# 3dlg-hcvc/tricolo

Measured on AMD Instinct MI355X. Metric: trimodal training samples/sec (32^3 voxel + 6-view), higher is better.
Workload: dtype f16 (f16 activation storage + f16 MFMA operands, fp32 accumulate; bf16x3 heads/GRU; within 1e-3 of the fp32 reference)

## Files before the change

### tricolo_amd/csrc/conv_igemm.hip

```cpp
#include "common.h"
#include <stdio.h>
#include <stdlib.h>
#include <map>
#include <mutex>
#include "../../include/tricolo_hip.h"
#include "conv_vox.h"
#include "conv_frag.h"

struct ConvArgs {
    const void* in;
    const void* w_hi;
    const void* w_lo;
    void* out;
    const uint8_t* row_mask;
    const int* row_pos;
    const int* row_count;
    const float* bias;
    float* stats;
    float* slab;
    int B, ID, IH, IW, Cin;
    int OD, OH, OW, Cout;
    int KD, KH, KW, stride, pd, ph, pw;
    int transposed, act, accumulate;
    int Kpad, M, ntaps, cin_shift, ksplit, steps_per_split;
// ... 1248 lines not shown
    HR_FIRST_READS(0u)
    HSTAMP(3);

#pragma unroll 1
    for (;;) {
        const int ng = grp_n(c_g);
        const bool last_chunk = c_chunk == nchunks - 1;
        HR_ELEM(0)
        HR_ELEM(1)
        HR_ELEM(2)
        HR_ELEM(3)
        int n_g = c_g, n_chunk = c_chunk + 1;
        if (n_chunk == nchunks) { n_chunk = 0; n_g += NTLE; }
        if (n_g >= n_my) break;
        if (!STREAM && !w_once) {
            asm volatile("s_waitcnt lgkmcnt(0)" ::: "memory");
            __builtin_amdgcn_s_barrier();
            asm volatile("" ::: "memory");
            w_row_pieces(n_chunk, 0, 0, 6);
            w_row_pieces(n_chunk, 1, 0, 6);
            w_row_pieces(n_chunk, 2, 0, 6);
            asm volatile("s_waitcnt vmcnt(0)" ::: "memory");
            __builtin_amdgcn_s_barrier();
            asm volatile("" ::: "memory");
            const unsigned sb0 = c_sbuf * slab_bytes;
            HR_FIRST_READS(sb0)
        }
        c_g = n_g; c_chunk = n_chunk;
    }
    asm volatile("s_waitcnt lgkmcnt(0)" ::: "memory");
    if (DRIP && d_on) {
#pragma unroll
        for (int d = 0; d < 4; ++d) {
            const v4i q = *(const v4i*)((const char*)red + wave * 4096 + (d >> 1) * 2048 + ((d & 1) * 8 + (lane >> 3)) * 128 +
                                        (((lane & 7) ^ ((((d & 1) * 8 + (lane >> 3)) >> 1) & 7)) << 4));
            if (d_m0 + d * 8 < d_npos) *(v4i*)(d_ptr + d * d_step) = q;
        }
    }
    __syncthreads();
    if (p.stats) halo_store_stats<TN, BN>(cs, cq, red, p.stats, p.Cout, bid / NT, bid % NT, wave, fr, fq, t, false);
    HSTAMP(11);
#ifdef HALO_STAMPS
    if (wave == 0) {
        asm volatile("s_waitcnt lgkmcnt(0)" ::: "memory");
        for (int i = lane; i < 255; i += 64) p.h_dbg[(size_t)blockIdx.x * 256 + i] = i < n_stamp ? stl[i] : 0;
        if (lane == 0) p.h_dbg[(size_t)blockIdx.x * 256 + 255] = n_stamp;
    }
#endif
#undef HR_ELEM
#undef HR_FIRST_READS
#undef HR_ROW
#undef HR_DRIP_READ
#undef HR_DRIP_STORE
#undef HR_KSTEP
#undef HR_MMA
}


#define STEM_MAX_KH 8
struct StemGeom { int TH, slab_rows, row_bytes, ptiles, tiles_per_img, ntiles, grid, npt; };
template <int KH, int NPT, typename AT>
__global__ __launch_bounds__(256, NPT == 2 ? 2 : 1) void conv_stem_kernel(const ConvArgs p, const StemGeom sg) {
    typedef Mma<typename OpOf<AT>::E> MM;
    typedef typename MM::v8 v8;
    extern __shared__ __attribute__((aligned(16))) char smem[];
    const int t = threadIdx.x, lane = t & 63, wave = __builtin_amdgcn_readfirstlane(t >> 6), fr = lane & 15, fq = lane >> 4;
    const int slab_bytes = sg.slab_rows * sg.row_bytes;
    float* const red = (float*)(smem + 2 * slab_bytes);
    const int OW = p.OW, IW = p.IW, IH = p.IH, OH = p.OH;
    const int pt_per_row = OW >> 4;

    v8 wf[KH][4];
    {
        const uint16_t* w = (const uint16_t*)p.w_hi;
#pragma unroll
        for (int kh = 0; kh < KH; ++kh)
#pragma unroll
            for (int ct = 0; ct < 4; ++ct) {
                const uint16_t* src = w + (size_t)(ct * 16 + fr) * p.Kpad + (kh * p.KW + 2 * fq) * 4;
                uint2 lo = make_uint2(0u, 0u), hi = make_uint2(0u, 0u);
                if (2 * fq < p.KW) lo = *(const uint2*)src;
                if (2 * fq + 1 < p.KW) hi = *(const uint2*)(src + 4);
                const uint4 raw = make_uint4(lo.x, lo.y, hi.x, hi.y);
                wf[kh][ct] = __builtin_bit_cast(v8, raw);
            }
        asm volatile("s_waitcnt vmcnt(0)" ::: "memory");
#pragma unroll
        for (int kh = 0; kh < KH; ++kh)
#pragma unroll
            for (int ct = 0; ct < 4; ++ct) asm volatile("" : "+v"(wf[kh][ct]));
    }
    for (int i = t * 16; i < 2 * slab_bytes; i += 256 * 16) *(uint4*)(smem + i) = make_uint4(0u, 0u, 0u, 0u);
    __syncthreads();

    constexpr int MAXLD = 4;
    const int ld_per_row = IW >> 1, nld = sg.slab_rows * ld_per_row;
    int ld_row[MAXLD], ld_goff[MAXLD], ld_loff[MAXLD];
#pragma unroll
    for (int u = 0; u < MAXLD; ++u) {
        const int e = t + u * 256;
        const int srow = e / ld_per_row, xp = e - srow * ld_per_row;
        ld_row[u] = e < nld ? srow : -(1 << 20);
        ld_goff[u] = (srow * IW + 2 * xp) * 8;
        ld_loff[u] = srow * sg.row_bytes + (2 * xp + p.pw) * 8;
    }
    uint4 pre[MAXLD];
    auto fetch = [&](int tile) {
        const int img = tile / sg.tiles_per_img, oh0 = (tile - img * sg.tiles_per_img) * sg.TH;
        const int iy0 = oh0 * 2 - p.ph;
        const char* base = (const char*)p.in + ((size_t)img * IH + iy0) * IW * 8;
#pragma unroll
        for (int u = 0; u < MAXLD; ++u) {
            pre[u] = make_uint4(0u, 0u, 0u, 0u);
            if ((unsigned)(iy0 + ld_row[u]) < (unsigned)IH) pre[u] = *(const uint4*)(base + ld_goff[u]);
        }
    };
    auto stash = [&](int buf) {
        char* sb = smem + buf * slab_bytes;
#pragma unroll
        for (int u = 0; u < MAXLD; ++u)
            if (ld_row[u] >= 0) {
                char* d = sb + ld_loff[u];
                *(uint2*)d = make_uint2(pre[u].x, pre[u].y);
                *(uint2*)(d + 8) = make_uint2(pre[u].z, pre[u].w);
            }
    };

    f32x4 cs[4], cq[4];
#pragma unroll
    for (int ct = 0; ct < 4; ++ct) { cs[ct] = (f32x4){0.f, 0.f, 0.f, 0.f}; cq[ct] = cs[ct]; }
    int boff[NPT], ooff[NPT], orow[NPT];
    bool inside[NPT];
#pragma unroll
    for (int j = 0; j < NPT; ++j) {
        const int q = wave + 4 * j;
        const int qc = q < sg.ptiles ? q : 0;
        const int r = qc / pt_per_row, c0 = (qc - r * pt_per_row) * 16;
        inside[j] = q < sg.ptiles;
        orow[j] = r;
        boff[j] = (2 * r) * sg.row_bytes + (c0 + fr + fq) * 16;
        ooff[j] = ((r * OW) + c0 + fr) * p.Cout + fq * 4;
    }

    int tile = blockIdx.x, buf = 0;
    if (tile < sg.ntiles) { fetch(tile); stash(0); }
    __syncthreads();
    for (; tile < sg.ntiles; tile += gridDim.x) {
        const int nxt = tile + gridDim.x;
        if (nxt < sg.ntiles && !(p.h_abl & 8)) fetch(nxt);
        const char* sb = smem + buf * slab_bytes;
        const int img = tile / sg.tiles_per_img, oh0 = (tile - img * sg.tiles_per_img) * sg.TH;
        f32x4 acc[NPT][4];
#pragma unroll
        for (int j = 0; j < NPT; ++j)
#pragma unroll
            for (int ct = 0; ct < 4; ++ct) acc[j][ct] = (f32x4){0.f, 0.f, 0.f, 0.f};
        if (!(p.h_abl & 1))
#pragma unroll
        for (int kh = 0; kh < KH; ++kh) {
            v8 b[NPT];
#pragma unroll
            for (int j = 0; j < NPT; ++j) b[j] = *(const v8*)(sb + boff[j] + kh * sg.row_bytes);
#pragma unroll
            for (int j = 0; j < NPT; ++j)
#pragma unroll
                for (int ct = 0; ct < 4; ++ct) acc[j][ct] = MM::mma(wf[kh][ct], b[j], acc[j][ct]);
        }
        AT* const obase = (AT*)p.out + ((size_t)img * OH + oh0) * OW * p.Cout;
#pragma unroll
        for (int j = 0; j < NPT; ++j) {
            if (inside[j] && oh0 + orow[j] < OH) {
                AT* o = obase + ooff[j];
#pragma unroll
                for (int ct = 0; ct < 4; ++ct) {
                    f32x4 v = acc[j][ct];
                    if (!(p.h_abl & 4)) Act<AT>::st4(o + ct * 16, make_float4(v[0], v[1], v[2], v[3]));
                    if (p.stats) {
                        v[0] = Act<AT>::rnd(v[0]); v[1] = Act<AT>::rnd(v[1]); v[2] = Act<AT>::rnd(v[2]); v[3] = Act<AT>::rnd(v[3]);
                        cs[ct] += v;
                        cq[ct] += v * v;
                    }
                }
            }
        }
        if (nxt < sg.ntiles) stash(buf ^ 1);
        __syncthreads();
        buf ^= 1;
    }
    if (p.stats) {
#pragma unroll
        for (int ct = 0; ct < 4; ++ct)
#pragma unroll
            for (int r = 0; r < 4; ++r) {
                float s_ = cs[ct][r], q_ = cq[ct][r];
                stat_row_sum(s_, q_);
                stat_stage(red, wave, 64, ct * 16 + fq * 4 + r, fr, s_, q_);
            }
        __syncthreads();
        if (t < 64) {
            float s_, q_;
            stat_wave_sum<4>(red, 0, 64, t, s_, q_);
            stat_store(p.stats, blockIdx.x, p.Cout, 0, t, s_, q_);
        }
    }
}

template <typename AT>
__global__ __launch_bounds__(256) void conv_splitk_finish_kernel(const ConvArgs p) {
    __shared__ float red[16][64][2];
    const int t = threadIdx.x, tc = t & 15, rl = t >> 4;
    const int chunk = blockIdx.x, m0 = chunk * 32, n = blockIdx.y * 64 + tc * 4;
    float4 s4 = make_float4(0.f, 0.f, 0.f, 0.f), q4 = s4;
    const float4 bv = p.bias ? *(const float4*)(p.bias + n) : make_float4(0.f, 0.f, 0.f, 0.f);
    const int Meff = p.row_count ? min(*p.row_count, p.M) : p.M;
#pragma unroll
    for (int rr = 0; rr < 2; ++rr) {
        int m = m0 + rl * 2 + rr;
        if (m >= Meff) continue;
        const size_t pos = p.row_pos ? (size_t)p.row_pos[m] : (size_t)m;
        bool live = p.row_mask ? (p.row_mask[pos] != 0) : true;
        float4 v = make_float4(0.f, 0.f, 0.f, 0.f);
        if (live) {
            const float* sp = p.slab + (size_t)m * p.Cout + n;
            const size_t zs = (size_t)p.M * p.Cout;
            int z = 0;
            for (; z + 4 <= p.ksplit; z += 4) {
                const float4 x0 = *(const float4*)(sp + (size_t)z * zs), x1 = *(const float4*)(sp + (size_t)(z + 1) * zs);
                const float4 x2 = *(const float4*)(sp + (size_t)(z + 2) * zs), x3 = *(const float4*)(sp + (size_t)(z + 3) * zs);
                v.x += x0.x; v.y += x0.y; v.z += x0.z; v.w += x0.w;
                v.x += x1.x; v.y += x1.y; v.z += x1.z; v.w += x1.w;
                v.x += x2.x; v.y += x2.y; v.z += x2.z; v.w += x2.w;
                v.x += x3.x; v.y += x3.y; v.z += x3.z; v.w += x3.w;
            }
            for (; z < p.ksplit; ++z) {
                const float4 x = *(const float4*)(sp + (size_t)z * zs);
                v.x += x.x; v.y += x.y; v.z += x.z; v.w += x.w;
            }
            v.x += bv.x; v.y += bv.y; v.z += bv.z; v.w += bv.w;
            if (p.act == 1) { v.x = fmaxf(v.x, 0.f); v.y = fmaxf(v.y, 0.f); v.z = fmaxf(v.z, 0.f); v.w = fmaxf(v.w, 0.f); }
            else if (p.act == 2) { v.x = tanhf(v.x); v.y = tanhf(v.y); v.z = tanhf(v.z); v.w = tanhf(v.w); }
        }
        AT* o = (AT*)p.out + pos * p.Cout + n;
        if (p.accumulate) { float4 e = Act<AT>::ld4(o); v.x += e.x; v.y += e.y; v.z += e.z; v.w += e.w; }
        Act<AT>::st4(o, v);
        if (sizeof(AT) == 2) v = make_float4(Act<AT>::rnd(v.x), Act<AT>::rnd(v.y), Act<AT>::rnd(v.z), Act<AT>::rnd(v.w));
        s4.x += v.x; s4.y += v.y; s4.z += v.z; s4.w += v.w;
        q4.x += v.x * v.x; q4.y += v.y * v.y; q4.z += v.z * v.z; q4.w += v.w * v.w;
    }
    if (p.stats) {
        float* d = &red[rl][tc * 4][0];
        d[0] = s4.x; d[1] = q4.x; d[2] = s4.y; d[3] = q4.y; d[4] = s4.z; d[5] = q4.z; d[6] = s4.w; d[7] = q4.w;
        __syncthreads();
        if (t < 64) {
            float s = 0.f, q = 0.f;
#pragma unroll
            for (int w = 0; w < 16; ++w) { s += red[w][t][0]; q += red[w][t][1]; }
            p.stats[((size_t)chunk * 2 + 0) * p.Cout + blockIdx.y * 64 + t] = s;
            p.stats[((size_t)chunk * 2 + 1) * p.Cout + blockIdx.y * 64 + t] = q;
        }
    }
}

__device__ __forceinline__ void prep_store(bool f16, uint16_t* hi, bf16_t* lo, size_t idx, float v) {
    if (f16) { hi[idx] = __builtin_bit_cast(uint16_t, (f16_t)v); return; }
    const bf16_t h = (bf16_t)v;
    hi[idx] = __builtin_bit_cast(uint16_t, h);
    if (lo) lo[idx] = (bf16_t)(v - (float)h);
}

__device__ __forceinline__ size_t prep_index(bool frag, int row, int k, int kpad) {
    if (!frag) return (size_t)row * kpad + k;
    return ((size_t)(row >> 4) * (kpad >> 5) + (k >> 5)) * 512 + ((((k & 31) >> 3) * 16 + (row & 15)) << 3) + (k & 7);
}

__device__ __forceinline__ void prep_store4(bool f16, uint16_t* hi, bf16_t* lo, size_t idx, float4 v) {
    if (f16) {
        f16x4 h;
        h[0] = (f16_t)v.x; h[1] = (f16_t)v.y; h[2] = (f16_t)v.z; h[3] = (f16_t)v.w;
        *(f16x4*)(hi + idx) = h;
        return;
    }
    bf16x4 h;
    h[0] = (bf16_t)v.x; h[1] = (bf16_t)v.y; h[2] = (bf16_t)v.z; h[3] = (bf16_t)v.w;
    *(bf16x4*)(hi + idx) = h;
    if (lo) {
        bf16x4 l;
        l[0] = (bf16_t)(v.x - (float)h[0]); l[1] = (bf16_t)(v.y - (float)h[1]); l[2] = (bf16_t)(v.z - (float)h[2]); l[3] = (bf16_t)(v.w - (float)h[3]);
        *(bf16x4*)(lo + idx) = l;
    }
}

__global__ void weight_prep_kernel(const float* __restrict__ w, long s_row, long s_tap, long s_inner, int rows, int ntaps,
                                   int inner, int inner_pad, int Kpad, uint16_t* __restrict__ hi, bf16_t* __restrict__ lo, int f16, int frag) {
    long idx = (long)blockIdx.x * blockDim.x + threadIdx.x;
    long total = (long)rows * Kpad;
    if (idx >= total) return;
    int row = (int)(idx / Kpad), k = (int)(idx - (long)row * Kpad);
    int tap = k / inner_pad, i = k - tap * inner_pad;
    float v = 0.f;
    if (tap < ntaps && i < inner) v = w[row * s_row + tap * s_tap + i * s_inner];
    prep_store(f16 != 0, hi, lo, prep_index(frag != 0, row, k, Kpad), v);
}

__global__ __launch_bounds__(256) void weight_prep_multi_kernel(const TriPrepDesc* __restrict__ descs) {
    __shared__ float tile[64 * 73];
    const TriPrepDesc d = descs[blockIdx.y];
    uint16_t* hi = (uint16_t*)d.hi;
    bf16_t* lo = (bf16_t*)d.lo;
    const bool f16 = d.fmt == TRI_FMT_F16, frag = d.frag != 0;
    const int t = threadIdx.x, nt = d.ntaps;
    const long span = (long)d.inner * nt;
    if (nt > 1 && d.s_tap == 1 && d.s_inner == nt && d.s_row == span && span <= 64 * 73 && d.inner == d.inner_pad) {
        const bool vec = (span & 3) == 0 && (d.inner_pad & 3) == 0 && (d.kpad & 3) == 0 && (((uintptr_t)d.w) & 15) == 0;
        for (int row = blockIdx.x; row < d.rows; row += gridDim.x) {
            const float* src = d.w + (size_t)row * d.s_row;
            if (vec) {
                for (int e = t * 4; e < span; e += 1024) *(float4*)(tile + e) = *(const float4*)(src + e);
                __syncthreads();
                for (int k = t * 4; k < d.kpad; k += 1024) {
                    const int tap = k / d.inner_pad, i = k - tap * d.inner_pad;
                    float4 v = make_float4(0.f, 0.f, 0.f, 0.f);
                    if (tap < nt) v = make_float4(tile[i * nt + tap], tile[(i + 1) * nt + tap], tile[(i + 2) * nt + tap], tile[(i + 3) * nt + tap]);
                    prep_store4(f16, hi, lo, prep_index(frag, row, k, d.kpad), v);
                }
            } else {
                for (int e = t; e < span; e += 256) tile[e] = src[e];
                __syncthreads();
                for (int k = t; k < d.kpad; k += 256) {
                    const int tap = k / d.inner_pad, i = k - tap * d.inner_pad;
                    prep_store(f16, hi, lo, prep_index(frag, row, k, d.kpad), tap < nt ? tile[i * nt + tap] : 0.f);
                }
            }
            __syncthreads();
        }
        return;
    }
    if (d.s_inner == 1 && d.s_tap == d.inner && d.s_row == span && d.inner == d.inner_pad && (span & 3) == 0 && (d.kpad & 3) == 0 &&
        (((uintptr_t)d.w) & 15) == 0) {
        const unsigned q4 = (unsigned)(d.kpad >> 2), total4 = (unsigned)d.rows * q4, used = (unsigned)span;
        for (unsigned e = blockIdx.x * 256u + t; e < total4; e += gridDim.x * 256u) {
            const unsigned row = e / q4, k = (e - row * q4) * 4u;
            float4 v = make_float4(0.f, 0.f, 0.f, 0.f);
            if (k < used) v = *(const float4*)(d.w + (size_t)row * span + k);
            prep_store4(f16, hi, lo, prep_index(frag, (int)row, (int)k, d.kpad), v);
        }
        return;
    }
    const bool torch_t = nt > 1 && nt <= 9 && d.s_tap == 1 && d.s_row == nt && d.s_inner == (long)d.rows * nt;
    const bool plane_t = d.s_row == 1 && d.s_tap == d.rows && d.s_inner == (long)d.rows * nt;
    if ((torch_t || plane_t) && d.inner == d.inner_pad) {
        const int RT = torch_t ? 8 : 32;
        const int run = torch_t ? RT * nt : RT, ld = run + 1;
        const int planes = torch_t ? 1 : nt;
        const int rtiles = (d.rows + RT - 1) / RT, itiles = (d.inner + 63) / 64;
        const long ntile = (long)rtiles * itiles * planes;
        for (long tl = blockIdx.x; tl < ntile; tl += gridDim.x) {
            const int plane = (int)(tl / ((long)rtiles * itiles));
            const int rem = (int)(tl - (long)plane * rtiles * itiles);
            const int r0 = (rem / itiles) * RT, i0 = (rem % itiles) * 64;
            const int rows_here = min(RT, d.rows - r0);
            const int run_here = torch_t ? rows_here * nt : rows_here;
            for (int e = t; e < 64 * run; e += 256) {
                const int il = e / run, r = e - il * run;
                float v = 0.f;
                if (i0 + il < d.inner && r < run_here)
                    v = d.w[(size_t)(i0 + il) * d.s_inner + (torch_t ? (size_t)r0 * nt + r : (size_t)plane * d.s_tap + r0 + r)];
                tile[il * ld + r] = v;
            }
            __syncthreads();
            if ((d.inner & 3) == 0 && (d.inner_pad & 3) == 0 && (d.kpad & 3) == 0) {
                for (int e = t; e < 16 * run; e += 256) {
                    const int il = (e & 15) * 4, r = e >> 4;
                    const int row_l = torch_t ? r / nt : r, tap = torch_t ? r - row_l * nt : plane;
                    if (row_l < rows_here && i0 + il < d.inner)
                        prep_store4(f16, hi, lo, prep_index(frag, r0 + row_l, tap * d.inner_pad + i0 + il, d.kpad),
                                    make_float4(tile[il * ld + r], tile[(il + 1) * ld + r], tile[(il + 2) * ld + r], tile[(il + 3) * ld + r]));
                }
            } else
            for (int e = t; e < 64 * run; e += 256) {
                const int il = e & 63, r = e >> 6;
                const int row_l = torch_t ? r / nt : r, tap = torch_t ? r - row_l * nt : plane;
                if (row_l < rows_here && i0 + il < d.inner)
                    prep_store(f16, hi, lo, prep_index(frag, r0 + row_l, tap * d.inner_pad + i0 + il, d.kpad), tile[il * ld + r]);
            }
            __syncthreads();
        }
        const int kused = nt * d.inner_pad, padw = d.kpad - kused;
        if (padw > 0)
            for (long e = (long)blockIdx.x * 256 + t; e < (long)d.rows * padw; e += (long)gridDim.x * 256) {
                const int row = (int)(e / padw), k = kused + (int)(e - (long)row * padw);
                prep_store(f16, hi, lo, prep_index(frag, row, k, d.kpad), 0.f);
            }
        return;
    }
    const long total = (long)d.rows * d.kpad;
    for (long idx = (long)blockIdx.x * blockDim.x + threadIdx.x; idx < total; idx += (long)gridDim.x * blockDim.x) {
        int row = (int)(idx / d.kpad), k = (int)(idx - (long)row * d.kpad);
        int tap = k / d.inner_pad, i = k - tap * d.inner_pad;
        float v = 0.f;
        if (tap < d.ntaps && i < d.inner) v = d.w[row * d.s_row + tap * d.s_tap + i * d.s_inner];
        prep_store(f16, hi, lo, prep_index(frag, row, k, d.kpad), v);
    }
}

extern "C" int tri_weight_prep_multi(const TriPrepDesc* descs_dev, int n, void* stream) {
    if (n <= 0) return TRI_OK;
    static int gx = 0;
    if (!gx) gx = 512;
    weight_prep_multi_kernel<<<dim3(gx, n), 256, 0, (hipStream_t)stream>>>(descs_dev);
    return tri_check_launch("tri_weight_prep_multi");
}

extern "C" int tri_weight_prep(const float* w, long s_row, long s_tap, long s_inner, int rows, int ntaps, int inner,
                               int inner_pad, void* w_hi, void* w_lo, int fmt, int frag, void* stream) {
    if (fmt == TRI_FMT_F16 && w_lo) { tri_set_error("tri_weight_prep: the f16 operand format has no lo part"); return TRI_ERR_ARG; }
    if (inner_pad % 4 != 0 || inner > inner_pad) { tri_set_error("tri_weight_prep: inner_pad must be a multiple of 4 >= inner"); return TRI_ERR_ARG; }
    if (frag && rows % 16 != 0) { tri_set_error("tri_weight_prep: the fragment-major order needs rows % 16 == 0"); return TRI_ERR_ARG; }
    int Kpad = (ntaps * inner_pad + 31) / 32 * 32;
    long total = (long)rows * Kpad;
    int blocks = (int)((total + 255) / 256);
    weight_prep_kernel<<<blocks, 256, 0, (hipStream_t)stream>>>(w, s_row, s_tap, s_inner, rows, ntaps, inner, inner_pad, Kpad,
                                                                (uint16_t*)w_hi, (bf16_t*)w_lo, fmt == TRI_FMT_F16 ? 1 : 0, frag ? 1 : 0);
    return tri_check_launch("tri_weight_prep");
}


template <int BN, int NSPLIT, typename AT>
static int launch_conv(const ConvArgs& a, hipStream_t stream) {
    constexpr int STAGE = NSPLIT * (128 * 64 + BN * 64);
    constexpr int WAVES_M = (BN >= 64) ? 2 : 4;
    size_t smem = 2 * STAGE + 512 + WAVES_M * BN * 2 * sizeof(float);
    static bool attr_set = false;
    if (!attr_set) {
        hipFuncSetAttribute((const void*)conv_igemm_kernel<BN, NSPLIT, AT>, hipFuncAttributeMaxDynamicSharedMemorySize, (int)smem);
        attr_set = true;
    }
    int mt = (a.M + 127) / 128, nt = a.Cout / BN;
    conv_igemm_kernel<BN, NSPLIT, AT><<<dim3(mt * nt, a.ksplit), 256, smem, stream>>>(a);
    int rc = tri_check_launch("tri_conv");
    if (rc || a.ksplit == 1) return rc;
    conv_splitk_finish_kernel<AT><<<dim3((a.M + 31) / 32, a.Cout / 64), 256, 0, stream>>>(a);
    return tri_check_launch("tri_conv_splitk_finish");
}

static int conv_bn(int cout) { return cout % 128 == 0 ? 128 : (cout % 64 == 0 ? 64 : 32); }

static TriConvDesc conv_view(const TriConvDesc& d, int transposed) {
    if (!transposed) return d;
    TriConvDesc v = d;
    v.ID = d.OD; v.IH = d.OH; v.IW = d.OW; v.Cin = d.Cout;
    v.OD = d.ID; v.OH = d.IH; v.OW = d.IW; v.Cout = d.Cin;
    return v;
}
static int conv_kpad(const TriConvDesc& v) { return (v.KD * v.KH * v.KW * v.Cin + 31) / 32 * 32; }

struct HaloGeom {
    int TM, tr, rows, slab_bytes, nr, mtiles, dbuf;
    int v5;
    int grid;
    int wgrec;
    int nt;
};

struct ConvFamily;
struct ConvPlan {
    const ConvFamily* family;
    unsigned fall_also;
    union {
        TriVox0Geom vox0; TriVoxbGeom voxb; TriVoxgGeom voxg; StemGeom stem; TriPwGeom pw; TriC64Geom c64; TriS2gGeom s2g;
    } g;
    HaloGeom halo;
    const ConvFamily* also;
    TriC64Geom also_g;
    int tile, spu;
    int dma;
    int bn;
    int nunits;
    int ksplit, per_split;
};

static int conv_target_blocks() {
    static int v = -1;
    if (v < 0) v = 0;
    return v;
}

static int num_cus() {
    static int v = 0;
    if (!v) {
        int dev = 0;
        hipDeviceProp_t pr;
        if (hipGetDevice(&dev) == hipSuccess && hipGetDeviceProperties(&pr, dev) == hipSuccess && pr.multiProcessorCount > 0) v = pr.multiProcessorCount;
        else v = 256;
    }
    return v;
}

int tri_internal_num_cus() { return num_cus(); }

static bool halo_geometry(const TriConvDesc& d, int TM, HaloGeom* pl) {
    const int B = d.B, H = d.IH, W = d.IW, cin = d.Cin, cout = d.Cout;
    const int BM = 64 * TM, P = W + 2;
    if (W > BM) return false;
    const int TR = BM / W;
    int k;
    if (H % TR == 0) k = 1;
    else if (TR % H == 0) k = TR / H;
    else return false;
    const int rows = TR + 2 * k;
    const int slab = ((rows * P + 1) * 128 + 4095) / 4096 * 4096;
    if (slab / 4096 > 10) return false;
    pl->TM = TM; pl->tr = TR; pl->rows = rows; pl->slab_bytes = slab; pl->nr = 3; pl->dbuf = 0;
    pl->mtiles = (B * H + TR - 1) / TR;
    pl->nt = cout / 64;
    {
        const int NT = pl->nt, items = pl->mtiles * NT;
        const size_t smem = (size_t)slab + (size_t)HALO_NR * 8192 + 2048;
        int per_cu = (int)(163840 / (smem + 256));
        per_cu = per_cu < 1 ? 1 : (per_cu > 3 ? 3 : per_cu);
        int slots = num_cus() * per_cu / NT * NT;
        if (slots < NT) slots = NT;
        pl->grid = items < slots ? items : slots;
        pl->wgrec = items >= 4 * slots ? 1 : 0;
        const int rows_kernel = tri_env_int("TRICOLO_HALO_ROWS", 1);
        pl->v5 = 0;
        int g = num_cus() / NT * NT;
        if (g < NT) g = NT;
        static int half_tiles = -1;
        if (half_tiles < 0) half_tiles = 3;
        static int deep = -1;
        if (deep < 0) deep = 1;
        if (rows_kernel && (cin == 64 || (deep && cin >= 256) || 2 * items <= half_tiles * g || rows_kernel == 2) && (TM == 2 || (TM == 3 && cin != 64)) &&
            2 * (size_t)slab + 3 * (size_t)HROWS_SLOT + 8192 <= 163840) {
            pl->v5 = 1;
            pl->grid = items < g ? items : g;
            pl->wgrec = 1;
        }
    }
    return true;
}

static bool stem_geometry(const TriConvDesc& d, StemGeom* g) {
    if (tri_env_is("TRICOLO_NO_STEM", '1') || d.ID != 1 || d.OD != 1) return false;
    const int B = d.B, IH = d.IH, IW = d.IW, OH = d.OH, OW = d.OW, KH = d.KH;
    if (d.KD != 1 || d.pad_d != 0 || d.Cin != 4 || d.stride != 2 || d.Cout != 64 || (KH != 3 && KH != 5 && KH != 7) || d.KW > 8 || OW % 16 || IW % 2) return false;
    if (d.pad_w < 0 || d.pad_h < 0 || IW + d.pad_w > 2 * OW + 6 || (long)B * IH * IW * 8 >= ((long)1 << 31)) return false;
    const int per_row = OW / 16;
    static int npt = -1;
    if (npt < 0) npt = 2;
    if (per_row > 4 * npt) return false;
    int TH = 4 * npt / per_row;
    if (TH > OH) TH = OH;
    g->npt = npt;
    g->TH = TH;
    g->slab_rows = (TH - 1) * 2 + KH;
    g->row_bytes = (OW + 3) * 16;
    g->ptiles = TH * per_row;
    g->tiles_per_img = (OH + TH - 1) / TH;
    g->ntiles = B * g->tiles_per_img;
    if (g->slab_rows * (IW / 2) > 256 * 4) return false;
    if (2 * g->slab_rows * g->row_bytes + 4 * 64 * 2 * 4 > 160 * 1024 / 2) return false;
    const int slots = num_cus() * (npt == 4 ? 1 : 2);
    g->grid = g->ntiles < slots ? g->ntiles : slots;
    return true;
}

static int dma_stages_for(const ConvArgs& a, int bn) {
    const int forced = tri_env_int("TRICOLO_DMA_STAGES", 0), rows = tri_env_int("TRICOLO_DMA_STAGES_ROWS", 0);
    if (forced >= 2 && forced <= 4) return forced;
    if (a.row_count && rows >= 2 && rows <= 4) return rows;
    const long wgs = (long)((a.M + 127) / 128) * (a.Cout / bn) * a.ksplit;
    const bool small = a.row_count != nullptr || wgs <= 2L * num_cus();
    return (small && bn <= 64) ? 3 : 2;
}

template <int BN, int NST, typename AT>
static int launch_dma(const ConvArgs& a, hipStream_t stream) {
    constexpr size_t smem = NST * (128 * 128 + BN * 128) + 512 + (size_t)4 * BN * 2 * sizeof(float);
    static bool attr = false;
    if (!attr) {
        hipFuncSetAttribute((const void*)conv_dma_kernel<BN, NST, AT>, hipFuncAttributeMaxDynamicSharedMemorySize, (int)smem);
        attr = true;
    }
    int mt = (a.M + 127) / 128, nt = a.Cout / BN;
    conv_dma_kernel<BN, NST, AT><<<dim3(mt * nt, a.ksplit), 256, smem, stream>>>(a);
    int rc = tri_check_launch("tri_conv(dma)");
    if (rc || a.ksplit == 1) return rc;
    conv_splitk_finish_kernel<AT><<<dim3((a.M + 31) / 32, a.Cout / 64), 256, 0, stream>>>(a);
    return tri_check_launch("tri_conv_splitk_finish");
}

static int halo_swizzle(int W, int H, int TM) {
    static std::mutex mu;
    static std::map<long, int> memo;
    if (W < 1 || H < 1 || TM < 1) return 0;
    const long key = ((long)TM << 40) | ((long)W << 20) | (long)H;
    {
        std::lock_guard<std::mutex> lk(mu);
        auto it = memo.find(key);
        if (it != memo.end()) return it->second;
    }
    static const int grp[4][16] = {{0, 1, 2, 3, 12, 13, 14, 15, 20, 21, 22, 23, 24, 25, 26, 27}, {4, 5, 6, 7, 8, 9, 10, 11, 16, 17, 18, 19, 28, 29, 30, 31},
                                   {32, 33, 34, 35, 44, 45, 46, 47, 52, 53, 54, 55, 56, 57, 58, 59}, {36, 37, 38, 39, 40, 41, 42, 43, 48, 49, 50, 51, 60, 61, 62, 63}};
    const int P = W + 2, TR = 64 * TM / W, whole = (TR % H == 0);
    long best = -1;
    int best_c = 0;
    for (int c1 = 0; c1 < 8; ++c1) {
        long cyc = 0;
        for (int wave = 0; wave < 4; ++wave)
            for (int a = 0; a < TM; ++a)
                for (int tap = 0; tap < 9; ++tap)
                    for (int kk = 0; kk < 2; ++kk)
                        for (int g = 0; g < 4; ++g) {
                            int cnt[16] = {0}, mx = 0;
                            for (int l = 0; l < 16; ++l) {
                                const int lane = grp[g][l], fr = lane & 15, fq = lane >> 4;
                                const int pa = wave * 16 * TM + a * 16 + fr, j = pa / W, x = pa - j * W, i = whole ? j / H : 0;
                                const int row = j + 1 + 2 * i + tap / 3 - 1, col = x + 1 + tap % 3 - 1;
                                const int slot = (((row * P + col) & 1) << 3) | (((fq + 4 * kk) ^ (col + c1 * row)) & 7);
                                if (++cnt[slot] > mx) mx = cnt[slot];
                            }
                            cyc += mx;
                        }
        if (best < 0 || cyc < best) { best = cyc; best_c = c1; }
    }
    std::lock_guard<std::mutex> lk(mu);
    memo[key] = best_c;
    return best_c;
}

#ifdef HALO_STAMPS
static long long* g_halo_dbg = nullptr;
#endif
template <int TM, typename AT>
static int launch_halo(ConvArgs& a, const HaloGeom& pl, hipStream_t stream) {
    a.h_tr = pl.tr; a.h_rows = pl.rows; a.h_slab_bytes = pl.slab_bytes; a.h_nr = pl.nr; a.h_mtiles = pl.mtiles;
    a.h_dbuf = pl.dbuf;
    a.h_abl = tri_probe_ablation();
    a.row_pos = nullptr;
    a.dP = make_fastdiv(a.IW + 2); a.dH2 = make_fastdiv(a.IH + 2);
    a.h_swz = halo_swizzle(a.IW, a.IH, pl.TM);
#ifdef HALO_STAMPS
    a.h_dbg = g_halo_dbg;
    const size_t smem = (size_t)pl.slab_bytes + (size_t)HALO_NR * 8192 + 2048 + 2048;
#else
    const size_t smem = (size_t)pl.slab_bytes + (size_t)HALO_NR * 8192 + 2048;
#endif
    a.h_xcg = 0; a.h_touch = 0;
    if (pl.v5) {
        const int xcg_env = tri_env_int("TRICOLO_HALO_XCG", -1), xcg_on = xcg_env < 0 ? 99 : xcg_env;
        const int touch_on = tri_env_is("TRICOLO_HALO_TOUCH", '0') ? 0 : 1;
        const int NT = a.Cout / 64, G = pl.grid;
        if (xcg_on && G == pl.mtiles * NT && G % 8 == 0 && a.Cin != 64) {
            const double wb = (double)a.Cout * a.Kpad * 2, ib = (double)a.M * a.Cin * 2;
            double best = 0;
            for (int cg = 1; cg <= NT; ++cg) {
                if (NT % cg || 8 % (NT / cg) || (G / 8) % cg) continue;
                if (xcg_on != 99 && cg != xcg_on) continue;
                const double bytes = wb * (8.0 * cg / NT) + ib * (NT / cg);
                if (!a.h_xcg || bytes < best) { a.h_xcg = cg; best = bytes; }
            }
            a.h_touch = a.h_xcg ? touch_on : 0;
        }
#ifdef HALO_STAMPS
        a.h_dbg = g_halo_dbg;
        const size_t extra = 2048;
#else
        const size_t extra = 0;
#endif
        const bool drip = 2 * (size_t)pl.slab_bytes + 3 * (size_t)HROWS_SLOT + 16384 + extra <= 163840 && !a.accumulate && pl.TM != 3;
        const size_t smem5 = 2 * (size_t)pl.slab_bytes + 3 * (size_t)HROWS_SLOT + (drip ? 16384 : 8192) + extra;
        int ntl = a.Cin == 64 ? 1 : 0;
#ifdef HALO_NTL_EXPERIMENT
        { static int f = -1; if (f < 0) f = 0;
          const int items = pl.mtiles * (a.Cout / 64), per_wg = (items + pl.grid - 1) / pl.grid;
          if (f && a.Cin != 64 && per_wg > 1) ntl = per_wg == 2 ? 2 : 4; }
#endif
#define TRI_ROWS_LAUNCH(DRIP_, ACC_, NTL_, ...)                                                                                     \
        do {                                                                                                                        \
            static size_t attr5 = 0;                                                                                                \
            if (smem5 > attr5) {                                                                                                    \
                hipFuncSetAttribute((const void*)conv_halo_rows_kernel<AT, DRIP_, ACC_, NTL_, ##__VA_ARGS__>, hipFuncAttributeMaxDynamicSharedMemorySize, \
                                    (int)smem5);                                                                                    \
                attr5 = smem5;                                                                                                      \
            }                                                                                                                       \
            conv_halo_rows_kernel<AT, DRIP_, ACC_, NTL_, ##__VA_ARGS__><<<pl.grid, 256, smem5, stream>>>(a);                       \
        } while (0)
#define TRI_ROWS_MODE(NTL_)                                                                                                         \
        do {                                                                                                                        \
            if (a.accumulate) TRI_ROWS_LAUNCH(false, true, NTL_);                                                                   \
            else if (drip) TRI_ROWS_LAUNCH(true, false, NTL_);                                                                      \
            else TRI_ROWS_LAUNCH(false, false, NTL_);                                                                               \
        } while (0)
        const bool prod = !tri_env_is("TRICOLO_HALO_PROD", '0');
        if (prod && pl.TM == 2 && ntl == 0) {
#define TRI_ROWS_LAUNCH_P(DRIP_, ACC_)                                                                                              \
        do {                                                                                                                        \
            static size_t attrp = 0;                                                                                                \
            if (smem5 > attrp) {                                                                                                    \
                hipFuncSetAttribute((const void*)conv_halo_rows_kernel<AT, DRIP_, ACC_, 0, 2, true>, hipFuncAttributeMaxDynamicSharedMemorySize, \
                                    (int)smem5);                                                                                    \
                attrp = smem5;                                                                                                      \
            }                                                                                                                       \
            conv_halo_rows_kernel<AT, DRIP_, ACC_, 0, 2, true><<<pl.grid, 512, smem5, stream>>>(a);                                \
        } while (0)
            if (a.accumulate) TRI_ROWS_LAUNCH_P(false, true);
            else if (drip) TRI_ROWS_LAUNCH_P(true, false);
            else TRI_ROWS_LAUNCH_P(false, false);
#undef TRI_ROWS_LAUNCH_P
            return tri_check_launch("tri_conv(halo rows, producer waves)");
        }
        if (pl.TM == 3) {
// ... 427 lines not shown
```

Measured before the change: 12950.

## Restructure multi-descriptor weight prep into flat tiled work queue with vectorized paths

```diff
diff --git a/tricolo_amd/csrc/conv_igemm.hip b/tricolo_amd/csrc/conv_igemm.hip
--- a/tricolo_amd/csrc/conv_igemm.hip
+++ b/tricolo_amd/csrc/conv_igemm.hip
@@ -1574,112 +1574,278 @@
     prep_store(f16 != 0, hi, lo, prep_index(frag != 0, row, k, Kpad), v);
 }
 
-__global__ __launch_bounds__(256) void weight_prep_multi_kernel(const TriPrepDesc* __restrict__ descs) {
-    __shared__ float tile[64 * 73];
-    const TriPrepDesc d = descs[blockIdx.y];
+enum { PREP_GENERIC = 0, PREP_CAST, PREP_FWD9, PREP_DG9, PREP_DG1 };
+constexpr int PREP_DG_LD = 33;
+constexpr int PREP_LDS_WORDS = 32 * 9 * PREP_DG_LD;
+constexpr int PREP_FWD_LD = 73;
+constexpr int PREP_GENERIC_TILE = 256, PREP_CAST_TILE = 4096;
+constexpr int PREP_FWD_BATCH = 5;
+
+__device__ __forceinline__ int prep_fwd9_rows(int inner) {
+    const int i8n = inner >> 3;
+    return max(1, min(PREP_FWD_BATCH * 1024 / (i8n * 72), PREP_LDS_WORDS / (i8n * PREP_FWD_LD)));
+}
+
+struct PrepWork { int path; long tiles; };
+
+__device__ __forceinline__ PrepWork prep_classify(const TriPrepDesc& d) {
+    PrepWork w;
+    const int nt = d.ntaps;
+    const long span = (long)d.inner * nt;
+    w.path = PREP_GENERIC;
+    w.tiles = ((long)d.rows * d.kpad + PREP_GENERIC_TILE - 1) / PREP_GENERIC_TILE;
+    if (d.rows <= 0 || d.inner <= 0 || nt <= 0) { w.tiles = d.rows > 0 ? w.tiles : 0; return w; }
+    const bool wide = ((((uintptr_t)d.hi) | ((uintptr_t)d.lo)) & 15) == 0 && (d.kpad & 7) == 0 && d.inner == d.inner_pad;
+    if (!wide) return w;
+    if (d.s_inner == 1 && (nt == 1 || d.s_tap == d.inner) && d.s_row == span && (span & 7) == 0) {
+        w.path = PREP_CAST;
+        w.tiles = ((long)d.rows * (d.kpad >> 3) * 8 + PREP_CAST_TILE - 1) / PREP_CAST_TILE;
+        return w;
+    }
+    if ((d.inner & 7) != 0) return w;
+    if (nt == 9 && d.s_tap == 1 && d.s_inner == 9 && d.s_row == span && (d.inner >> 3) * PREP_FWD_LD <= PREP_LDS_WORDS) {
+        const int R = prep_fwd9_rows(d.inner);
+        w.path = PREP_FWD9;
+        w.tiles = (d.rows + R - 1) / R;
+        return w;
+    }
+    if ((d.rows & 3) != 0) return w;
+    const long rtiles = (d.rows + 31) >> 5, itiles = (d.inner + 63) >> 6;
+    if (nt == 9 && d.s_tap == 1 && d.s_row == 9 && d.s_inner == (long)d.rows * 9) {
+        w.path = PREP_DG9;
+        w.tiles = rtiles * itiles;
+        return w;
+    }
+    if (d.s_row == 1 && d.s_inner == (long)d.rows * nt && (nt == 1 || d.s_tap == d.rows)) {
+        w.path = PREP_DG1;
+        w.tiles = rtiles * itiles * nt;
+        return w;
+    }
+    return w;
+}
+
+__device__ __forceinline__ uint16_t prep_hi16(bool f16, float v) {
+    return f16 ? __builtin_bit_cast(uint16_t, (f16_t)v) : __builtin_bit_cast(uint16_t, (bf16_t)v);
+}
+__device__ __forceinline__ uint16_t prep_lo16(float v) {
+    const bf16_t h = (bf16_t)v;
+    return __builtin_bit_cast(uint16_t, (bf16_t)(v - (float)h));
+}
+__device__ __forceinline__ uint32_t prep_pair(uint16_t a, uint16_t b) { return (uint32_t)a | ((uint32_t)b << 16); }
+
+typedef float prep_f4 __attribute__((ext_vector_type(4)));
+typedef uint32_t prep_u4 __attribute__((ext_vector_type(4)));
+#define PREP_GLOBAL __attribute__((address_space(1)))
+
+__device__ __forceinline__ void prep_st16(void* arr, size_t idx, uint32_t a, uint32_t b, uint32_t c, uint32_t e) {
+    prep_u4 v;
+    v[0] = a; v[1] = b; v[2] = c; v[3] = e;
+    *(PREP_GLOBAL prep_u4*)((PREP_GLOBAL uint16_t*)arr + idx) = v;
+}
+
+__device__ __forceinline__ void prep_store8(bool f16, uint16_t* hi, bf16_t* lo, size_t idx, const float (&v)[8]) {
+    prep_st16(hi, idx, prep_pair(prep_hi16(f16, v[0]), prep_hi16(f16, v[1])), prep_pair(prep_hi16(f16, v[2]), prep_hi16(f16, v[3])),
+              prep_pair(prep_hi16(f16, v[4]), prep_hi16(f16, v[5])), prep_pair(prep_hi16(f16, v[6]), prep_hi16(f16, v[7])));
+    if (lo)
+        prep_st16(lo, idx, prep_pair(prep_lo16(v[0]), prep_lo16(v[1])), prep_pair(prep_lo16(v[2]), prep_lo16(v[3])),
+                  prep_pair(prep_lo16(v[4]), prep_lo16(v[5])), prep_pair(prep_lo16(v[6]), prep_lo16(v[7])));
+}
+
+template <bool AL>
+__device__ __forceinline__ float4 prep_ld4(const float* p) {
+    const PREP_GLOBAL float* g = (const PREP_GLOBAL float*)p;
+    if (AL) { const prep_f4 v = *(const PREP_GLOBAL prep_f4*)g; return make_float4(v[0], v[1], v[2], v[3]); }
+    return make_float4(g[0], g[1], g[2], g[3]);
+}
+
+template <bool AL>
+__device__ __forceinline__ void prep_cast_tile(const TriPrepDesc& d, long tl, int t) {
+    const unsigned k8 = (unsigned)(d.kpad >> 3), used = (unsigned)(d.inner * d.ntaps), pieces = (unsigned)d.rows * k8;
+    constexpr int U = PREP_CAST_TILE / 8 / 256;
+    unsigned row[U], k[U];
+    float4 a[U], b[U];
+#pragma unroll
+    for (int u = 0; u < U; ++u) {
+        const unsigned c = min((unsigned)tl * (PREP_CAST_TILE / 8) + u * 256 + t, pieces - 1);
+        row[u] = c / k8; k[u] = (c - row[u] * k8) * 8u;
+        const float* p = d.w + (size_t)row[u] * used + min(k[u], used - 8u);
+        a[u] = prep_ld4<AL>(p); b[u] = prep_ld4<AL>(p + 4);
+    }
+#pragma unroll
+    for (int u = 0; u < U; ++u) {
+        if ((unsigned)tl * (PREP_CAST_TILE / 8) + u * 256 + t >= pieces) break;
+        const bool in = k[u] < used;
+        const float v[8] = {in ? a[u].x : 0.f, in ? a[u].y : 0.f, in ? a[u].z : 0.f, in ? a[u].w : 0.f,
+                            in ? b[u].x : 0.f, in ? b[u].y : 0.f, in ? b[u].z : 0.f, in ? b[u].w : 0.f};
+        prep_store8(d.fmt == TRI_FMT_F16, (uint16_t*)d.hi, (bf16_t*)d.lo, prep_index(d.frag != 0, (int)row[u], (int)k[u], d.kpad), v);
+    }
+}
+
+template <bool AL>
+__device__ __forceinline__ void prep_fwd9_tile(const TriPrepDesc& d, long tl, int t, uint32_t* lds) {
+    float* stage = (float*)lds;
+    const unsigned i8n = (unsigned)(d.inner >> 3), span = (unsigned)d.inner * 9u;
+    const int R = prep_fwd9_rows(d.inner);
+    const int row0 = (int)tl * R, rows_here = min(R, d.rows - row0);
+    const float* src = d.w + (size_t)row0 * span;
+    const int n4 = rows_here * (int)(span >> 2);
+    for (int e0 = t; e0 < n4; e0 += PREP_FWD_BATCH * 256) {
+        float4 x[PREP_FWD_BATCH];
+#pragma unroll
+        for (int u = 0; u < PREP_FWD_BATCH; ++u) x[u] = prep_ld4<AL>(src + (size_t)min(e0 + u * 256, n4 - 1) * 4);
+#pragma unroll
+        for (int u = 0; u < PREP_FWD_BATCH; ++u) {
+            const int e = (e0 + u * 256) * 4;
+            if (e0 + u * 256 < n4) {
+                float* q = stage + e + e / 72;
+                q[0] = x[u].x; q[1] = x[u].y; q[2] = x[u].z; q[3] = x[u].w;
+            }
+        }
+    }
+    __syncthreads();
+    const bool f16 = d.fmt == TRI_FMT_F16, frag = d.frag != 0;
     uint16_t* hi = (uint16_t*)d.hi;
     bf16_t* lo = (bf16_t*)d.lo;
+    const unsigned pieces = (unsigned)rows_here * 9u * i8n;
+    for (unsigned c = t; c < pieces; c += 256) {
+        const unsigned rt = c / i8n, i8 = c - rt * i8n;
+        const unsigned row_l = rt / 9u, tap = rt - row_l * 9u;
+        const float* q = stage + (row_l * i8n + i8) * PREP_FWD_LD + tap;
+        float v[8];
+#pragma unroll
+        for (int m = 0; m < 8; ++m) v[m] = q[m * 9];
+        prep_store8(f16, hi, lo, prep_index(frag, row0 + (int)row_l, (int)(tap * d.inner + i8 * 8u), d.kpad), v);
+    }
+    const unsigned padc = (unsigned)(d.kpad - (int)span) >> 3;
+    if (padc) {
+        const float z[8] = {0.f, 0.f, 0.f, 0.f, 0.f, 0.f, 0.f, 0.f};
+        for (unsigned c = t; c < (unsigned)rows_here * padc; c += 256) {
+            const unsigned row_l = c / padc, pc = c - row_l * padc;
+            prep_store8(f16, hi, lo, prep_index(frag, row0 + (int)row_l, (int)(span + pc * 8u), d.kpad), z);
+        }
+    }
+    __syncthreads();
+}
+
+struct PrepDgTile { const float* src; unsigned s_in; int r0, rows_here, cos_here, run4, kbase, tap_k, kpad; bool frag; };
+
+template <int CVT>
+__device__ __forceinline__ uint16_t prep_cvt(float v) {
+    if (CVT == 1) return __builtin_bit_cast(uint16_t, (f16_t)v);
+    if (CVT == 2) return prep_lo16(v);
+    return __builtin_bit_cast(uint16_t, (bf16_t)v);
+}
+
+template <int NT, bool AL, int CVT>
+__device__ __forceinline__ void prep_dgrad_pass(const PrepDgTile& g, uint16_t* dst, int t, uint32_t* lds) {
+    const int lane = t & 63, wave = t >> 6, chunk = lane & 7, cosub = lane >> 3;
+    uint16_t* l16 = (uint16_t*)lds;
+#pragma unroll(NT == 1 ? 2 : 1)
+    for (int half = 0; half < 2; ++half) {
+        const int co = (half * 4 + wave) * 8 + cosub;
+        const unsigned co_off = (unsigned)min(co, g.cos_here - 1) * g.s_in;
+        float4 x[NT];
+#pragma unroll
+        for (int ln = 0; ln < NT; ++ln)
+            x[ln] = prep_ld4<AL>(g.src + (co_off + (unsigned)min(ln * 8 + chunk, g.run4 - 1) * 4u));
+        uint16_t* p = l16 + chunk * 4 * (2 * PREP_DG_LD) + co;
+#pragma unroll
+        for (int ln = 0; ln < NT; ++ln) {
+            uint16_t* pl = p + ln * 32 * (2 * PREP_DG_LD);
+            pl[0] = prep_cvt<CVT>(x[ln].x); pl[2 * PREP_DG_LD] = prep_cvt<CVT>(x[ln].y);
+            pl[4 * PREP_DG_LD] = prep_cvt<CVT>(x[ln].z); pl[6 * PREP_DG_LD] = prep_cvt<CVT>(x[ln].w);
+        }
+    }
+    __syncthreads();
+    const int ci_l = t >> 3, c8 = t & 7;
+    if (ci_l < g.rows_here && c8 * 8 < g.cos_here) {
+#pragma unroll
+        for (int tap = 0; tap < NT; ++tap) {
+            const uint32_t* s = lds + (ci_l * NT + tap) * PREP_DG_LD + c8 * 4;
+            prep_st16(dst, prep_index(g.frag, g.r0 + ci_l, tap * g.tap_k + g.kbase + c8 * 8, g.kpad), s[0], s[1], s[2], s[3]);
+        }
+    }
+    __syncthreads();
+}
+
+template <int NT, bool AL>
+__device__ __forceinline__ void prep_dgrad_tile(const TriPrepDesc& d, long tl, int t, uint32_t* lds) {
+    const int rtiles = (d.rows + 31) >> 5, itiles = (d.inner + 63) >> 6;
+    const int plane = (int)(tl / ((long)rtiles * itiles));
+    const int rem = (int)(tl - (long)plane * rtiles * itiles);
+    const int rt = rem / itiles, r0 = rt * 32, i0 = (rem - rt * itiles) * 64;
+    PrepDgTile g;
+    g.r0 = r0; g.rows_here = min(32, d.rows - r0); g.cos_here = min(64, d.inner - i0);
+    g.run4 = g.rows_here * NT >> 2;
+    const uintptr_t sa = (uintptr_t)(d.w + (size_t)i0 * d.s_inner + (NT == 1 ? (size_t)plane * d.rows : (size_t)0) + (size_t)r0 * NT);
+    g.src = (const float*)(((uintptr_t)(unsigned)__builtin_amdgcn_readfirstlane((int)(sa >> 32)) << 32) |
+                           (unsigned)__builtin_amdgcn_readfirstlane((int)(unsigned)sa));
+    g.s_in = (unsigned)d.s_inner;
+    g.kbase = (NT == 1 ? plane * d.inner_pad : 0) + i0; g.tap_k = d.inner_pad; g.kpad = d.kpad; g.frag = d.frag != 0;
+    const bool frag = g.frag;
+    const int rows_here = g.rows_here;
+    if (d.fmt == TRI_FMT_F16) prep_dgrad_pass<NT, AL, 1>(g, (uint16_t*)d.hi, t, lds);
+    else prep_dgrad_pass<NT, AL, 0>(g, (uint16_t*)d.hi, t, lds);
+    if (d.lo) prep_dgrad_pass<NT, AL, 2>(g, (uint16_t*)d.lo, t, lds);
+    const int kused = d.ntaps * d.inner_pad, padc = (d.kpad - kused) >> 3;
+    if (padc > 0 && i0 + 64 >= d.inner && plane == 0 && t < 128) {
+        const int row_l = t >> 2, pc = t & 3;
+        if (row_l < rows_here && pc < padc) {
+            const size_t idx = prep_index(frag, r0 + row_l, kused + pc * 8, d.kpad);
+            prep_st16(d.hi, idx, 0u, 0u, 0u, 0u);
+            if (d.lo) prep_st16(d.lo, idx, 0u, 0u, 0u, 0u);
+        }
+    }
+}
+
+__device__ __forceinline__ void prep_generic_tile(const TriPrepDesc& d, long tl, int t) {
+    const long total = (long)d.rows * d.kpad;
     const bool f16 = d.fmt == TRI_FMT_F16, frag = d.frag != 0;
-    const int t = threadIdx.x, nt = d.ntaps;
-    const long span = (long)d.inner * nt;
-    if (nt > 1 && d.s_tap == 1 && d.s_inner == nt && d.s_row == span && span <= 64 * 73 && d.inner == d.inner_pad) {
-        const bool vec = (span & 3) == 0 && (d.inner_pad & 3) == 0 && (d.kpad & 3) == 0 && (((uintptr_t)d.w) & 15) == 0;
-        for (int row = blockIdx.x; row < d.rows; row += gridDim.x) {
-            const float* src = d.w + (size_t)row * d.s_row;
-            if (vec) {
-                for (int e = t * 4; e < span; e += 1024) *(float4*)(tile + e) = *(const float4*)(src + e);
-                __syncthreads();
-                for (int k = t * 4; k < d.kpad; k += 1024) {
-                    const int tap = k / d.inner_pad, i = k - tap * d.inner_pad;
-                    float4 v = make_float4(0.f, 0.f, 0.f, 0.f);
-                    if (tap < nt) v = make_float4(tile[i * nt + tap], tile[(i + 1) * nt + tap], tile[(i + 2) * nt + tap], tile[(i + 3) * nt + tap]);
-                    prep_store4(f16, hi, lo, prep_index(frag, row, k, d.kpad), v);
-                }
-            } else {
-                for (int e = t; e < span; e += 256) tile[e] = src[e];
-                __syncthreads();
-                for (int k = t; k < d.kpad; k += 256) {
-                    const int tap = k / d.inner_pad, i = k - tap * d.inner_pad;
-                    prep_store(f16, hi, lo, prep_index(frag, row, k, d.kpad), tap < nt ? tile[i * nt + tap] : 0.f);
-                }
-            }
-            __syncthreads();
-        }
-        return;
-    }
-    if (d.s_inner == 1 && d.s_tap == d.inner && d.s_row == span && d.inner == d.inner_pad && (span & 3) == 0 && (d.kpad & 3) == 0 &&
-        (((uintptr_t)d.w) & 15) == 0) {
-        const unsigned q4 = (unsigned)(d.kpad >> 2), total4 = (unsigned)d.rows * q4, used = (unsigned)span;
-        for (unsigned e = blockIdx.x * 256u + t; e < total4; e += gridDim.x * 256u) {
-            const unsigned row = e / q4, k = (e - row * q4) * 4u;
-            float4 v = make_float4(0.f, 0.f, 0.f, 0.f);
-            if (k < used) v = *(const float4*)(d.w + (size_t)row * span + k);
-            prep_store4(f16, hi, lo, prep_index(frag, (int)row, (int)k, d.kpad), v);
-        }
-        return;
-    }
-    const bool torch_t = nt > 1 && nt <= 9 && d.s_tap == 1 && d.s_row == nt && d.s_inner == (long)d.rows * nt;
-    const bool plane_t = d.s_row == 1 && d.s_tap == d.rows && d.s_inner == (long)d.rows * nt;
-    if ((torch_t || plane_t) && d.inner == d.inner_pad) {
-        const int RT = torch_t ? 8 : 32;
-        const int run = torch_t ? RT * nt : RT, ld = run + 1;
-        const int planes = torch_t ? 1 : nt;
-        const int rtiles = (d.rows + RT - 1) / RT, itiles = (d.inner + 63) / 64;
-        const long ntile = (long)rtiles * itiles * planes;
-        for (long tl = blockIdx.x; tl < ntile; tl += gridDim.x) {
-            const int plane = (int)(tl / ((long)rtiles * itiles));
-            const int rem = (int)(tl - (long)plane * rtiles * itiles);
-            const int r0 = (rem / itiles) * RT, i0 = (rem % itiles) * 64;
-            const int rows_here = min(RT, d.rows - r0);
-            const int run_here = torch_t ? rows_here * nt : rows_here;
-            for (int e = t; e < 64 * run; e += 256) {
-                const int il = e / run, r = e - il * run;
-                float v = 0.f;
-                if (i0 + il < d.inner && r < run_here)
-                    v = d.w[(size_t)(i0 + il) * d.s_inner + (torch_t ? (size_t)r0 * nt + r : (size_t)plane * d.s_tap + r0 + r)];
-                tile[il * ld + r] = v;
-            }
-            __syncthreads();
-            if ((d.inner & 3) == 0 && (d.inner_pad & 3) == 0 && (d.kpad & 3) == 0) {
-                for (int e = t; e < 16 * run; e += 256) {
-                    const int il = (e & 15) * 4, r = e >> 4;
-                    const int row_l = torch_t ? r / nt : r, tap = torch_t ? r - row_l * nt : plane;
-                    if (row_l < rows_here && i0 + il < d.inner)
-                        prep_store4(f16, hi, lo, prep_index(frag, r0 + row_l, tap * d.inner_pad + i0 + il, d.kpad),
-                                    make_float4(tile[il * ld + r], tile[(il + 1) * ld + r], tile[(il + 2) * ld + r], tile[(il + 3) * ld + r]));
-                }
-            } else
-            for (int e = t; e < 64 * run; e += 256) {
-                const int il = e & 63, r = e >> 6;
-                const int row_l = torch_t ? r / nt : r, tap = torch_t ? r - row_l * nt : plane;
-                if (row_l < rows_here && i0 + il < d.inner)
-                    prep_store(f16, hi, lo, prep_index(frag, r0 + row_l, tap * d.inner_pad + i0 + il, d.kpad), tile[il * ld + r]);
-            }
-            __syncthreads();
-        }
-        const int kused = nt * d.inner_pad, padw = d.kpad - kused;
-        if (padw > 0)
-            for (long e = (long)blockIdx.x * 256 + t; e < (long)d.rows * padw; e += (long)gridDim.x * 256) {
-                const int row = (int)(e / padw), k = kused + (int)(e - (long)row * padw);
-                prep_store(f16, hi, lo, prep_index(frag, row, k, d.kpad), 0.f);
-            }
-        return;
-    }
-    const long total = (long)d.rows * d.kpad;
-    for (long idx = (long)blockIdx.x * blockDim.x + threadIdx.x; idx < total; idx += (long)gridDim.x * blockDim.x) {
+    for (int j = 0; j < PREP_GENERIC_TILE / 256; ++j) {
+        const long idx = tl * PREP_GENERIC_TILE + j * 256 + t;
+        if (idx >= total) return;
         int row = (int)(idx / d.kpad), k = (int)(idx - (long)row * d.kpad);
         int tap = k / d.inner_pad, i = k - tap * d.inner_pad;
         float v = 0.f;
         if (tap < d.ntaps && i < d.inner) v = d.w[row * d.s_row + tap * d.s_tap + i * d.s_inner];
-        prep_store(f16, hi, lo, prep_index(frag, row, k, d.kpad), v);
+        prep_store(f16, (uint16_t*)d.hi, (bf16_t*)d.lo, prep_index(frag, row, k, d.kpad), v);
+    }
+}
+
+__global__ __launch_bounds__(256, 4) void weight_prep_multi_kernel(const TriPrepDesc* __restrict__ descs, int n) {
+    __shared__ uint32_t lds[PREP_LDS_WORDS];
+    __shared__ unsigned count[256];
+    const int t = threadIdx.x;
+    long next = blockIdx.x, base = 0;
+    for (int d0 = 0; d0 < n; d0 += 256) {
+    if (d0) __syncthreads();
+    if (d0 + t < n) count[t] = (unsigned)prep_classify(descs[d0 + t]).tiles;
+    __syncthreads();
+    for (int di = d0; di < min(n, d0 + 256); ++di) {
+        const long tiles = (long)(unsigned)__builtin_amdgcn_readfirstlane((int)count[di - d0]);
+        if (next >= base + tiles) { base += tiles; continue; }
+        const TriPrepDesc d = descs[di];
+        const PrepWork w = prep_classify(d);
+        const bool al = (((uintptr_t)d.w) & 15) == 0;
+        for (; next < base + w.tiles; next += gridDim.x) {
+            const long tl = next - base;
+            switch (w.path) {
+            case PREP_CAST: if (al) prep_cast_tile<true>(d, tl, t); else prep_cast_tile<false>(d, tl, t); break;
+            case PREP_FWD9: if (al) prep_fwd9_tile<true>(d, tl, t, lds); else prep_fwd9_tile<false>(d, tl, t, lds); break;
+            case PREP_DG9:  if (al) prep_dgrad_tile<9, true>(d, tl, t, lds); else prep_dgrad_tile<9, false>(d, tl, t, lds); break;
+            case PREP_DG1:  if (al) prep_dgrad_tile<1, true>(d, tl, t, lds); else prep_dgrad_tile<1, false>(d, tl, t, lds); break;
+            default: prep_generic_tile(d, tl, t);
+            }
+        }
+        base += w.tiles;
+    }
     }
 }
 
 extern "C" int tri_weight_prep_multi(const TriPrepDesc* descs_dev, int n, void* stream) {
     if (n <= 0) return TRI_OK;
-    static int gx = 0;
-    if (!gx) gx = 512;
-    weight_prep_multi_kernel<<<dim3(gx, n), 256, 0, (hipStream_t)stream>>>(descs_dev);
+    const int grid = n < 16 ? 64 * n : 1024;
+    weight_prep_multi_kernel<<<grid, 256, 0, (hipStream_t)stream>>>(descs_dev, n);
     return tri_check_launch("tri_weight_prep_multi");
 }
 
```

Result: no change. 12860 (-0.7%).
